# jyakaranda/A-LeGO-LOAM

Measured on AMD Instinct MI355X. Metric: scans/sec (16x1800 LiDAR) full IP->LO->LM loop, higher is better.
Workload: dtype f32/f64

## Files before the change

a-lego-loam_amd/csrc/kernels_lm.hip:

```cpp
#include <cstddef>
#include <cstring>

#include "../../include/alego_mi355x.h"
#include "dev_cost.h"
#include "nn_rules.h"
#include "remap_math.h"
#include "prof.h"
#include "kf_store.h"
#include "gmap.h"
#include "vgrid.h"
#include "vox_merge.h"

#define LM_BLOCK 256

DEV_INLINE double* ldp(const LmCtx& L, int slot) { return L.ld + (size_t)slot * LD_COUNT; }
DEV_INLINE int* lip(const LmCtx& L, int slot) { return L.li + (size_t)slot * LI_COUNT; }

DEV_INLINE void lm_map_update(const LmCtx& L, int slot, int* li, int merge) {
  const int nkf = li[LI_NKF];
  if (nkf == 0) return;
  int* rec = L.rec + (size_t)slot * L.K;
  const int cnt = li[LI_REC_CNT];
  bool changed = false;
  if (cnt < L.K) {
// ... 243 lines not shown
        int tot;
        const int e = noo + block_excl_scan<LT_T / 64>(oh ? 1 : 0, s_w, &tot);
        if (j < no) s_oop[j] = e;
        noo += tot;
      }
      if (tid == 0) s_oop[no] = noo;
      __syncthreads();
      vm_u64 kprev = c0 > 0 && c0 < c1 ? vkey_of(S[c0 - 1], inv) : 0;
      int hl = 0;
      for (int b0 = c0; b0 < c1; b0 += LT_B) {
        float4 p[LT_B + 1];
#pragma unroll
        for (int k = 0; k <= LT_B; ++k) p[k] = S[min(b0 + k, ns - 1)];
#pragma unroll
        for (int k = 0; k < LT_B; ++k) {
          const int i = b0 + k;
          if (i < c1) {
            const vm_u64 key = vkey_of(p[k], inv);
            if (i == 0 || kprev != key) {
              const int ol = vm_count_less(s_skey, no, key), ole = vm_count_le(s_skey, no, key);
              const int r = base + hl + s_oop[ol];
              ++hl;
              if (r < cap) {
                int nsr = 1;
                if (i + 1 < ns && vkey_of(p[k + 1], inv) == key) while (i + nsr < ns && vkey_of(S[i + nsr], inv) == key) ++nsr;
                out[r] = vm_centroid([&](int q) { return q == 0 ? p[k] : (q < nsr ? S[i + q] : O[s_idx[ol + q - nsr]]); }, 0, nsr + ole - ol);
              }
            }
            kprev = key;
          }
        }
      }
      for (int j = tid; j < no; j += LT_T) {
        if (s_osb[j] >= 0 && (j == 0 || s_skey[j - 1] != s_skey[j])) {
          const int r = s_base[s_osb[j] >> 16] + (s_osb[j] & 0xFFFF) + s_oop[j];
          if (r < cap) {
            int e = j + 1;
            while (e < no && s_skey[e] == s_skey[j]) ++e;
            out[r] = vm_centroid([&](int q) { return O[s_idx[q]]; }, j, e);
          }
        }
      }
      const int nvox = nsh + noo;
      if (tid == 0) { li[LI_NTOTAL] = n; li[LI_NTOTAL_DS] = min(nvox, cap); if (nvox > cap) li[LI_OVERFLOW] = 1; li[LI_TM_FAST] += 1; }
    } else {
      float4* t = L.cur_total + (size_t)slot * L.total_cap;
      for (int i = tid; i < ns; i += LT_T) t[i] = S[i];
      for (int i = tid; i < no; i += LT_T) t[ns + i] = O[i];
      if (tid == 0) { li[LI_NTOTAL] = n; li[LI_TM_LIST] += 1; }
      state = n > W.small_max ? 2 : 1;
    }
  }
  if (tid == 0) {
    if (state == 1) W.list_small[atomicAdd(&W.cnt[0], 1)] = slot - L.vox_slot0;
    else if (state == 2) W.list_big[atomicAdd(&W.cnt[1], 1)] = slot - L.vox_slot0;
    if (blockIdx.x == 0) { W.cnt_next[0] = 0; W.cnt_next[1] = 0; }
  }
}

DEV_INLINE int grid_cell(const GridGeom& g, float x, float y, float z, int* cx, int* cy, int* cz) {
  *cx = nn_lm_coord(x, g.inv) - g.ox; *cy = nn_lm_coord(y, g.inv) - g.oy; *cz = nn_lm_coord(z, g.inv) - g.oz;
  return nn_lm_index(*cx, *cy, *cz, g.gx, g.gy, g.gz);
}

__global__ void __launch_bounds__(LM_BLOCK) lm_grid_build(DevCtx d, LmCtx L) {
  const int slot = blockIdx.y + d.slot0, m = blockIdx.x;
  const int* li = lip(L, slot);
  if (!li[LI_REBUILD]) return;
  __shared__ GridGeom s_g;
  __shared__ int s[LM_BLOCK / 64];
  __shared__ int s_run;
  if (threadIdx.x == 0) {
    const unsigned* bb = d.opt_map_merge ? L.map_bbox + ((size_t)slot * 2 + m) * 8 : L.vox_bbox + ((size_t)(slot - L.vox_slot0) * 2 + m) * 8;
    GridGeom g;
    float mn[3], mx[3];
    vgr_box_load(bb, mn, mx);
    if (li[LI_KRAW_C + m] <= 0) { for (int a = 0; a < 3; ++a) { mn[a] = 0.f; mx[a] = 0.f; } }
    float cell = nn_lm_cell(d.P.knn_max_dist);
    int lo[3], hi[3];
    for (;;) {
      for (int a = 0; a < 3; ++a) { lo[a] = nn_lm_coord(mn[a], 1.0f / cell) - 1; hi[a] = nn_lm_coord(mx[a], 1.0f / cell) + 1; }
      const long long ex = (long long)hi[0] - lo[0] + 1, ey = (long long)hi[1] - lo[1] + 1, ez = (long long)hi[2] - lo[2] + 1;
      if (ex <= L.gcap && ey <= L.gcap && ez <= L.gcap && ex * ey * ez <= (long long)L.gcap) { g.gx = (int)ex; g.gy = (int)ey; g.gz = (int)ez; break; }
      cell *= 2.0f;
    }
    g.ox = lo[0]; g.oy = lo[1]; g.oz = lo[2]; g.inv = 1.0f / cell; g.ncell = g.gx * g.gy * g.gz;
    s_g = g;
    L.grid[(size_t)slot * 2 + m] = g;
    s_run = 0;
  }
  __syncthreads();
  const GridGeom g = s_g;
  const int ncell = g.ncell;
  int* cs = L.cell_start + ((size_t)slot * 2 + m) * (L.gcap + 1);
  int* cc = L.cell_cur + ((size_t)slot * 2 + m) * (L.gcap + 1);
  for (int c = threadIdx.x; c <= ncell; c += LM_BLOCK) cs[c] = 0;
  __threadfence_block();
  __syncthreads();
  const int n = li[LI_KDS_C + m];
  const float4* pts = (m == 0 ? L.map_corner_ds + (size_t)slot * L.map_cap_c : L.map_surf_ds + (size_t)slot * L.map_cap_s);
  float4* cp = L.cell_pts + ((size_t)slot * 2 + m) * L.map_cap_s;
  for (int i = threadIdx.x; i < n; i += LM_BLOCK) {
    const float4 p = pts[i];
    int cx, cy, cz;
    atomicAdd(&cs[grid_cell(g, p.x, p.y, p.z, &cx, &cy, &cz)], 1);
  }
  __threadfence_block();
  __syncthreads();
  for (int c0 = 0; c0 <= ncell; c0 += LM_BLOCK) {
    const int c = c0 + threadIdx.x;
    const int v = __hip_atomic_load(&cs[min(c, ncell)], __ATOMIC_RELAXED, __HIP_MEMORY_SCOPE_AGENT) * (c < ncell ? 1 : 0);
    int tot;
    const int ex = block_excl_scan<LM_BLOCK / 64>(v, s, &tot);
    const int run = s_run;
    if (c <= ncell) { const int e2 = run + ex; cs[c] = e2; cc[c] = e2; }
    __syncthreads();
    if (threadIdx.x == 0) s_run = run + tot;
  }
  __threadfence_block();
  __syncthreads();
  for (int i = threadIdx.x; i < n; i += LM_BLOCK) {
    const float4 p = pts[i];
    int cx, cy, cz;
    const int pos = atomicAdd(&cc[grid_cell(g, p.x, p.y, p.z, &cx, &cy, &cz)], 1);
    cp[pos] = make_float4(p.x, p.y, p.z, __int_as_float(i));
  }
}

DEV_INLINE void d_eig3(const double Ain[9], double lam[3], double vmax[3], double* lam_mid) {
  double A[9], V[9];
#pragma unroll
  for (int i = 0; i < 9; ++i) { A[i] = Ain[i]; V[i] = (i % 4 == 0) ? 1.0 : 0.0; }
  for (int sweep = 0; sweep < 60; ++sweep) {
    const double off = A[1] * A[1] + A[2] * A[2] + A[5] * A[5];
    if (off < 1e-300) break;
    if (off <= 1e-40 * (A[0] * A[0] + A[4] * A[4] + A[8] * A[8])) break;
#pragma unroll
    for (int p = 0; p < 2; ++p)
#pragma unroll
      for (int q = p + 1; q < 3; ++q) {
        const double apq = A[p * 3 + q];
        if (apq == 0.0) continue;
        const double theta = (A[q * 3 + q] - A[p * 3 + p]) / (2.0 * apq);
        const double t = (theta >= 0 ? 1.0 : -1.0) / (fabs(theta) + sqrt(theta * theta + 1.0));
        const double c = 1.0 / sqrt(t * t + 1.0), s = t * c;
#pragma unroll
        for (int k = 0; k < 3; ++k) { const double akp = A[k * 3 + p], akq = A[k * 3 + q]; A[k * 3 + p] = c * akp - s * akq; A[k * 3 + q] = s * akp + c * akq; }
#pragma unroll
        for (int k = 0; k < 3; ++k) { const double apk = A[p * 3 + k], aqk = A[q * 3 + k]; A[p * 3 + k] = c * apk - s * aqk; A[q * 3 + k] = s * apk + c * aqk; }
#pragma unroll
        for (int k = 0; k < 3; ++k) { const double vkp = V[k * 3 + p], vkq = V[k * 3 + q]; V[k * 3 + p] = c * vkp - s * vkq; V[k * 3 + q] = s * vkp + c * vkq; }
      }
  }
  const double dd[3] = {A[0], A[4], A[8]};
  int imax = 0, imin = 0;
  if (dd[1] > dd[imax]) imax = 1;
  if (dd[2] > dd[imax]) imax = 2;
  if (dd[1] < dd[imin]) imin = 1;
  if (dd[2] < dd[imin]) imin = 2;
  int imid = 3 - imax - imin;
  if (imax == imin) { imax = 2; imin = 0; imid = 1; }
  lam[0] = dd[imin]; lam[1] = dd[imid]; lam[2] = dd[imax];
  *lam_mid = dd[imid];
  vmax[0] = V[0 * 3 + imax]; vmax[1] = V[1 * 3 + imax]; vmax[2] = V[2 * 3 + imax];
}

DEV_INLINE void d_colpiv_qr53(double A[3][5], const double b[5], double x[3]) {
  const double eps = 2.220446049250313e-16, tiny = 2.2250738585072014e-308;
  double nu[3], nd[3], hc[3], c[5];
  int perm[3] = {0, 1, 2};
  double maxn = 0;
#pragma unroll
  for (int k = 0; k < 3; ++k) {
    double s2 = 0;
#pragma unroll
    for (int i = 0; i < 5; ++i) s2 += A[k][i] * A[k][i];
    nd[k] = nu[k] = sqrt(s2);
    if (nu[k] > maxn) maxn = nu[k];
  }
  const double threshold_helper = (maxn * eps) * (maxn * eps) / 5.0;
  const double downdate_threshold = 1.4901161193847656e-08;
  int nonzero = 3;
#pragma unroll
  for (int k = 0; k < 3; ++k) {
    int big = k;
    double nbig = nu[k];
#pragma unroll
    for (int j = k + 1; j < 3; ++j) if (nu[j] > nbig) { big = j; nbig = nu[j]; }
    if (nonzero == 3 && nbig * nbig < threshold_helper * (double)(5 - k)) nonzero = k;
#pragma unroll
    for (int j = k + 1; j < 3; ++j)
      if (big == j) {
#pragma unroll
        for (int i = 0; i < 5; ++i) { const double t = A[k][i]; A[k][i] = A[j][i]; A[j][i] = t; }
        { const double t = nu[k]; nu[k] = nu[j]; nu[j] = t; }
        { const double t = nd[k]; nd[k] = nd[j]; nd[j] = t; }
        { const int t = perm[k]; perm[k] = perm[j]; perm[j] = t; }
      }
    double tail2 = 0;
#pragma unroll
    for (int i = k + 1; i < 5; ++i) tail2 += A[k][i] * A[k][i];
    const double c0 = A[k][k];
    double beta, tau;
    if (tail2 <= tiny) {
      tau = 0; beta = c0;
#pragma unroll
      for (int i = k + 1; i < 5; ++i) A[k][i] = 0;
    } else {
      beta = sqrt(c0 * c0 + tail2);
      if (c0 >= 0) beta = -beta;
#pragma unroll
      for (int i = k + 1; i < 5; ++i) A[k][i] = A[k][i] / (c0 - beta);
      tau = (beta - c0) / beta;
    }
    hc[k] = tau;
    A[k][k] = beta;
    if (tau != 0) {
#pragma unroll
      for (int j = k + 1; j < 3; ++j) {
        double t = 0;
#pragma unroll
        for (int i = k + 1; i < 5; ++i) t += A[k][i] * A[j][i];
        t += A[j][k];
        A[j][k] -= tau * t;
#pragma unroll
        for (int i = k + 1; i < 5; ++i) A[j][i] -= tau * A[k][i] * t;
      }
    }
#pragma unroll
    for (int j = k + 1; j < 3; ++j) {
      if (nu[j] != 0) {
        double t = fabs(A[j][k]) / nu[j];
        t = (1.0 + t) * (1.0 - t);
        t = t < 0 ? 0 : t;
        const double q = nu[j] / nd[j];
        const double t2 = t * (q * q);
        if (t2 <= downdate_threshold) {
          double s2 = 0;
#pragma unroll
          for (int i = k + 1; i < 5; ++i) s2 += A[j][i] * A[j][i];
          nd[j] = nu[j] = sqrt(s2);
        } else nu[j] *= sqrt(t);
      }
    }
  }
#pragma unroll
  for (int i = 0; i < 5; ++i) c[i] = b[i];
#pragma unroll
  for (int k = 0; k < 3; ++k) {
    const double tau = hc[k];
    if (k < nonzero && tau != 0) {
      double t = 0;
#pragma unroll
      for (int i = k + 1; i < 5; ++i) t += A[k][i] * c[i];
      t += c[k];
      c[k] -= tau * t;
#pragma unroll
      for (int i = k + 1; i < 5; ++i) c[i] -= tau * A[k][i] * t;
    }
  }
#pragma unroll
  for (int k = 2; k >= 0; --k) {
    if (k < nonzero) {
      double sum = c[k];
#pragma unroll
      for (int j = k + 1; j < 3; ++j) if (j < nonzero) sum -= A[j][k] * c[j];
      c[k] = sum / A[k][k];
    } else c[k] = 0.0;
  }
#pragma unroll
  for (int o = 0; o < 3; ++o) {
    double v = 0.0;
#pragma unroll
    for (int i = 0; i < 3; ++i) if (perm[i] == o) v = c[i];
    x[o] = v;
  }
}

#ifndef LM_KNN_LANES
#define LM_KNN_LANES 4
#endif

DEV_INLINE void lm_shard_slice(const LmCtx& L, int nqc, int nqs, int kind, int* qlo, int* qhi) {
  int lo = 0, hi = nqc + nqs;
  if (L.shard_world > 1) {
    const long long T = nqc + nqs;
    lo = (int)(T * L.shard_rank / L.shard_world); hi = (int)(T * (L.shard_rank + 1) / L.shard_world);
  }
  if (kind == 0) { *qlo = min(lo, nqc); *qhi = min(hi, nqc); } else { *qlo = max(lo - nqc, 0); *qhi = max(hi - nqc, 0); }
}

DEV_INLINE bool lm_reg_block(const DevCtx& d, int GX, int* slot, int* kind, int* bx) {
  const int per = 2 * GX, b = blockIdx.x, oct = b / (8 * per), r = b - oct * 8 * per;
  const int s = oct * 8 + (r & 7), w = r >> 3;
  *slot = s + d.slot0; *kind = w / GX; *bx = w - (w / GX) * GX;
  return s < d.n_launch;
}
static inline int lm_reg_grid(const DevCtx& d, int GX) { return ((d.n_launch + 7) / 8) * 8 * 2 * GX; }

#define LM_ASSOC_GX 64
#ifndef LM_KNN_PK
#define LM_KNN_PK 1
#endif
__global__ void __launch_bounds__(128) lm_knn(DevCtx d, LmCtx L) {
  int slot, kind, bx;
  if (!lm_reg_block(d, LM_ASSOC_GX, &slot, &kind, &bx)) return;
  const int gx = LM_ASSOC_GX;
  const int* li = lip(L, slot);
  if (!li[LI_RUN]) return;
  const alego_params& P = d.P;
  if (lm_reg_skipped(li, P)) return;
  const int nq = kind == 0 ? li[LI_NCUR_C] : li[LI_NTOTAL_DS];
  int qlo, qhi;
  lm_shard_slice(L, li[LI_NCUR_C], li[LI_NTOTAL_DS], kind, &qlo, &qhi);
  const float4* qp = kind == 0 ? L.cur_corner_ds + (size_t)slot * L.kf_cap_c : L.cur_total_ds + (size_t)slot * L.total_cap;
  const int nmap = li[LI_KDS_C + kind];
  const GridGeom g = L.grid[(size_t)slot * 2 + kind];
  const int* cs = L.cell_start + ((size_t)slot * 2 + kind) * (L.gcap + 1);
  const float4* cp = L.cell_pts + ((size_t)slot * 2 + kind) * L.map_cap_s;
  const double* ld = ldp(L, slot);
  const DQuat qm = ldq(ld + LD_Q_M2L);
  constexpr int QPB = 128 / LM_KNN_LANES;
  const int sub = threadIdx.x & (LM_KNN_LANES - 1);
  const uint32_t limbits = nn_lm_limit_bits(P.knn_max_dist);
  const int nq_round = (nq + QPB - 1) / QPB * QPB;
  for (int qq = bx * QPB + threadIdx.x / LM_KNN_LANES; qq < nq_round; qq += gx * QPB) {
  const int q = min(qq, nq - 1);
  const float4 pin = qp[q];
  const double vin[3] = {pin.x, pin.y, pin.z};
  double r[3];
  dq_rotate(qm, vin, r);
  const float sx = (float)(r[0] + ld[LD_T_M2L + 0]), sy = (float)(r[1] + ld[LD_T_M2L + 1]), sz = (float)(r[2] + ld[LD_T_M2L + 2]);
  typedef nn_key_t u64k;
  const u64k KNONE = NN_NONE;
  u64k k0 = KNONE, k1 = KNONE, k2 = KNONE, k3 = KNONE, k4 = KNONE, kmax = KNONE;
  if (nmap >= 5 && q >= qlo && q < qhi) {
    int cx, cy, cz;
    grid_cell(g, sx, sy, sz, &cx, &cy, &cz);
    int rs[9], re[9];
#pragma unroll
    for (int r = 0; r < 9; ++r) {
      const int z = cz + r / 3 - 1, y = cy + r % 3 - 1;
      const int x0 = max(cx - 1, 0), x1 = min(cx + 1, g.gx - 1);
      const bool in = z >= 0 && z < g.gz && y >= 0 && y < g.gy && x0 <= x1;
      const int c0 = x0 + g.gx * (y + g.gy * z), c1 = x1 + g.gx * (y + g.gy * z);
      const int a0 = cs[in ? c0 : 0], a1 = cs[in ? c1 + 1 : 0];
      rs[r] = in ? a0 : 0;
      re[r] = in ? a1 : 0;
    }
    const nn_v2f sxy = {sx, sy};
    auto consider = [&](const float4& a) {
#if LM_KNN_PK
      const float dist = nn_d2_pk(sxy, sz, nn_v2f{a.x, a.y}, a.z);
#else
      const float dist = nn_d2(sx, sy, sz, a.x, a.y, a.z);
#endif
      const u64k key = nn_key(dist, (uint32_t)__float_as_int(a.w));
      if (key < kmax && nn_lm_within(dist, limbits)) {
        const bool e0 = k0 == kmax, e1 = !e0 && k1 == kmax, e2 = !e0 && !e1 && k2 == kmax, e3 = !e0 && !e1 && !e2 && k3 == kmax, e4 = !e0 && !e1 && !e2 && !e3;
        k0 = e0 ? key : k0; k1 = e1 ? key : k1; k2 = e2 ? key : k2; k3 = e3 ? key : k3; k4 = e4 ? key : k4;
        const u64k m01 = k0 > k1 ? k0 : k1, m23 = k2 > k3 ? k2 : k3, m03 = m01 > m23 ? m01 : m23;
        kmax = m03 > k4 ? m03 : k4;
      }
    };
    float4 first[9];
#pragma unroll
    for (int r = 0; r < 9; ++r) first[r] = cp[rs[r] + sub < re[r] ? rs[r] + sub : 0];
#ifndef LM_KNN_ORDER
#define LM_KNN_ORDER 1
#endif
    constexpr int ord[9] = {4, 1, 3, 5, 7, 0, 2, 6, 8};
#pragma unroll
    for (int k = 0; k < 9; ++k) { const int r = LM_KNN_ORDER ? ord[k] : k; if (rs[r] + sub < re[r]) consider(first[r]); }
#pragma unroll
    for (int k = 0; k < 9; ++k) {
      const int r = LM_KNN_ORDER ? ord[k] : k;
      for (int t = rs[r] + sub + LM_KNN_LANES; t < re[r]; t += 2 * LM_KNN_LANES) {
        const int t1 = t + LM_KNN_LANES;
        const float4 a0 = cp[t], a1 = cp[t1 < re[r] ? t1 : t];
        consider(a0);
        if (t1 < re[r]) consider(a1);
      }
    }
  }
  float bd[5];
  int bi[5];
  {
#pragma unroll
    for (int k = 0; k < 5; ++k) {
      const u64k m01 = k0 < k1 ? k0 : k1, m23 = k2 < k3 ? k2 : k3, m03 = m01 < m23 ? m01 : m23, mine = m03 < k4 ? m03 : k4;
      const u64k m = group_min_u64<LM_KNN_LANES>(mine);
      bd[k] = nn_key_d2(m); bi[k] = nn_key_index(m);
      if (mine == m && m != KNONE) {
        k0 = k0 == m ? KNONE : k0; k1 = k1 == m ? KNONE : k1; k2 = k2 == m ? KNONE : k2; k3 = k3 == m ? KNONE : k3; k4 = k4 == m ? KNONE : k4;
      }
    }
  }
  if (sub == 0 && qq < nq) {
    int* kn = lm_knn_of(L, slot, kind, q);
    const bool ok = nn_lm_row_ok(bi[4], bd[4], P.knn_max_dist) && q >= qlo && q < qhi;
#pragma unroll
    for (int k = 0; k < 5; ++k) kn[k] = ok ? bi[k] : -1;
  }
  }
}

#define LM_FIT_GX 20
__global__ void __launch_bounds__(128) lm_fit(DevCtx d, LmCtx L) {
  int slot, kind, bx;
  if (!lm_reg_block(d, LM_FIT_GX, &slot, &kind, &bx)) return;
  const int gx = LM_FIT_GX;
  const int* li = lip(L, slot);
  if (!li[LI_RUN]) return;
  const alego_params& P = d.P;
  if (lm_reg_skipped(li, P)) return;
  const int nq = kind == 0 ? li[LI_NCUR_C] : li[LI_NTOTAL_DS];
  const float4* mp = kind == 0 ? L.map_corner_ds + (size_t)slot * L.map_cap_c : L.map_surf_ds + (size_t)slot * L.map_cap_s;
  for (int q = bx * 128 + threadIdx.x; q < nq; q += gx * 128) {
  const int* kn = lm_knn_of(L, slot, kind, q);
  double* blk = lm_blocks_of(L, slot) + lm_row_of(kind, q, L.kf_cap_c) * LMB_W;
  int bi[5];
#pragma unroll
  for (int k = 0; k < 5; ++k) bi[k] = kn[k];
  lmb_put_none(blk);
  do {
    if (bi[0] < 0) break;
  if (kind == 0) {
    double near[5][3], center[3] = {0, 0, 0};
#pragma unroll
    for (int j = 0; j < 5; ++j) {
      const float4 m = mp[bi[j]];
      near[j][0] = m.x; near[j][1] = m.y; near[j][2] = m.z;
#pragma unroll
      for (int a = 0; a < 3; ++a) center[a] = center[a] + near[j][a];
    }
#pragma unroll
    for (int a = 0; a < 3; ++a) center[a] = center[a] / 5.0;
    double cov[9] = {0, 0, 0, 0, 0, 0, 0, 0, 0};
#pragma unroll
    for (int j = 0; j < 5; ++j) {
      const double zm[3] = {near[j][0] - center[0], near[j][1] - center[1], near[j][2] - center[2]};
#pragma unroll
      for (int a = 0; a < 3; ++a)
#pragma unroll
        for (int b = 0; b < 3; ++b) cov[a * 3 + b] = cov[a * 3 + b] + zm[a] * zm[b];
    }
    double lam[3], v[3], lmid;
    d_eig3(cov, lam, v, &lmid);
    if (lam[2] > P.line_ratio * lam[1]) {
      double pa[3], pb[3];
#pragma unroll
      for (int a = 0; a < 3; ++a) { pa[a] = P.line_half_len * v[a] + center[a]; pb[a] = -P.line_half_len * v[a] + center[a]; }
      lmb_put_edge(blk, pa, pb);
    }
  } else {
    double A[3][5], b[5], nrm[3];
    float mx[5], my[5], mz[5];
#pragma unroll
    for (int j = 0; j < 5; ++j) {
      const float4 m = mp[bi[j]];
      mx[j] = m.x; my[j] = m.y; mz[j] = m.z;
      A[0][j] = m.x; A[1][j] = m.y; A[2][j] = m.z; b[j] = -1.0;
    }
    d_colpiv_qr53(A, b, nrm);
    const double nn = sqrt(nrm[0] * nrm[0] + nrm[1] * nrm[1] + nrm[2] * nrm[2]);
    const double dd = 1 / nn;
#pragma unroll
    for (int a = 0; a < 3; ++a) nrm[a] /= nn;
    bool ok = true;
#pragma unroll
    for (int j = 0; j < 5; ++j)
      if (fabs(nrm[0] * mx[j] + nrm[1] * my[j] + nrm[2] * mz[j] + dd) > P.plane_tol) ok = false;
    if (ok) lmb_put_plane(blk, nrm, dd);
  }
  } while (false);
  }
}

#ifndef LM_SOLVE_T
#define LM_SOLVE_T 256
#endif
#define LM_SOLVE_RED_BYTES ((size_t)28 * (LM_SOLVE_T / 8) * sizeof(double))
#define LM_SOLVE_DYN_BYTES ((size_t)158 * 1024)
#define LM_SOLVE_ROW_BYTES_DEFAULT ((size_t)96 * 1024)
template <int T>
DEV_INLINE void lm_pack_rows(const LmCtx& L, int slot, int nqc, int nqs, unsigned char* row_lds, size_t row_budget, int (*s_cnt)[T / 64], LmRows& W) {
  const int tid = threadIdx.x, lane = tid & 63, wave = tid >> 6;
  const double* blocks = lm_blocks_of(L, slot);
  const float4* qc = L.cur_corner_ds + (size_t)slot * L.kf_cap_c;
  const float4* qs = L.cur_total_ds + (size_t)slot * L.total_cap;
  const int n_all = nqc + nqs, per = (n_all + T - 1) / T;
  const int lo = min(tid * per, n_all), hi = min(lo + per, n_all);
  auto block_of = [&](int i) { return blocks + lm_row_of_query(i, nqc, L.kf_cap_c) * LMB_W; };
  constexpr int U = 4;
  int cc = 0, cs = 0;
  for (int i0 = lo; i0 < hi; i0 += U) {
    double ty[U];
#pragma unroll
    for (int u = 0; u < U; ++u) ty[u] = block_of(min(i0 + u, n_all - 1))[LMB_TYPE];
#pragma unroll
    for (int u = 0; u < U; ++u) if (i0 + u < hi && ty[u] != 0.0) { if (i0 + u < nqc) ++cc; else ++cs; }
  }
  const int ic = wave_incl_scan(cc), is = wave_incl_scan(cs);
  if (lane == 63) { s_cnt[0][wave] = ic; s_cnt[1][wave] = is; }
  __syncthreads();
  int epos = ic - cc, ppos = is - cs, Rc = 0, Rs = 0;
#pragma unroll
  for (int w = 0; w < T / 64; ++w) { const int a = s_cnt[0][w], b = s_cnt[1][w]; if (w < wave) { epos += a; ppos += b; } Rc += a; Rs += b; }
  W = lml_make(Rc, Rs, row_lds, row_budget, lm_crows_of(L, slot));
  for (int i0 = lo; i0 < hi; i0 += U) {
    LmBlock B[U];
    float4 pt[U];
#pragma unroll
    for (int u = 0; u < U; ++u) {
      const int i = min(i0 + u, n_all - 1);
      B[u] = lmb_load(block_of(i));
      pt[u] = i < nqc ? qc[i] : qs[i - nqc];
    }
#pragma unroll
    for (int u = 0; u < U; ++u) {
      const int i = i0 + u;
      if (i < hi && lmb_type(B[u]) != 0.0) {
        const bool is_c = i < nqc;
        const int r = is_c ? epos++ : ppos++;
        if (is_c && r < W.Ce) lml_put_edge(W, r, B[u], pt[u]);
        else if (!is_c && r < W.Cp) lml_put_plane(W, r, B[u], pt[u]);
        else lms_put(W.crows + (is_c ? lms_edge_at(r) : lms_plane_at(Rc, r)) * LMS_W, B[u], pt[u]);
      }
    }
  }
  __threadfence_block();
  __syncthreads();
}

template <int T, bool FULL = true>
DEV_INLINE void lm_eval_rows(const LmRows& W, const PoseTerms& Tm, double huber, double acc[28]) {
  const double c3[3] = {0, 0, 0};
  for (int i = threadIdx.x; i < W.Rc; i += T) {
    LmEdge e;
    if (i < W.Ce) e = lml_edge(W, i); else e = lms_edge(W.crows + lms_edge_at(i) * LMS_W);
    if constexpr (FULL) {
      double res, J[6];
      eval_block(BLK_EDGE, e.p, e.a, e.b, c3, 0.0, Tm, &res, J);
      accumulate_block(res, J, huber, acc);
    } else accumulate_cost(eval_block_residual<BLK_EDGE>(e.p, e.a, e.b, c3, 0.0, Tm), huber, acc[27]);
  }
  for (int j = threadIdx.x; j < W.Rs; j += T) {
    LmPlane p;
    if (j < W.Cp) p = lml_plane(W, j); else p = lms_plane(W.crows + lms_plane_at(W.Rc, j) * LMS_W);
    if constexpr (FULL) {
      double res, J[6];
      eval_block(BLK_PLANE, p.p, p.n, c3, c3, p.d, Tm, &res, J);
      accumulate_block(res, J, huber, acc);
    } else accumulate_cost(eval_block_residual<BLK_PLANE>(p.p, p.n, c3, c3, p.d, Tm), huber, acc[27]);
  }
}

struct ShflHip { DEV_INLINE double operator()(double v, int src) const { return __shfl(v, src); } };
struct ShflDirect {
  DEV_INLINE double operator()(double v, int src) const {
    const long long b = __double_as_longlong(v);
    const int lo = __builtin_amdgcn_ds_bpermute(src << 2, (int)(unsigned)(unsigned long long)b), hi = __builtin_amdgcn_ds_bpermute(src << 2, (int)(unsigned)((unsigned long long)b >> 32));
    return __longlong_as_double((long long)(((unsigned long long)(unsigned)hi << 32) | (unsigned)lo));
  }
};
template <class Shfl>
DEV_INLINE double rc_eigen_lanes(double A, int i, int j, double lam[6], const Shfl& shfl) {
  double V = i == j ? 1.0 : 0.0;
  for (int sweep = 0; sweep < RC_SWEEPS_MAX; ++sweep) {
    double off = 0.0, dg = 0.0;
#pragma unroll
    for (int a = 0; a < 6; ++a)
#pragma unroll
      for (int b = a + 1; b < 6; ++b) { const double x = shfl(A, a * 6 + b); off += x * x; }
#pragma unroll
    for (int a = 0; a < 6; ++a) { const double x = shfl(A, a * 7); dg += x * x; }
    if (!(off > RC_OFF_REL * dg)) break;
#pragma unroll
    for (int pp = 0; pp < 5; ++pp)
#pragma unroll
      for (int q = pp + 1; q < 6; ++q) {
        const double apq = shfl(A, pp * 6 + q);
        if (apq == 0.0) continue;
        double c, s;
        rc_rot_cs(shfl(A, pp * 7), shfl(A, q * 7), apq, &c, &s);
        { const double xp = shfl(A, i * 6 + pp), xq = shfl(A, i * 6 + q); A = rc_rot_col(j, pp, q, c, s, xp, xq, A); }
        { const double xp = shfl(A, pp * 6 + j), xq = shfl(A, q * 6 + j); A = rc_rot_row(i, pp, q, c, s, xp, xq, A); }
        { const double xp = shfl(V, i * 6 + pp), xq = shfl(V, i * 6 + q); V = rc_rot_col(j, pp, q, c, s, xp, xq, V); }
      }
  }
  double dd[6];
  int rk[6], src = 0;
#pragma unroll
  for (int k = 0; k < 6; ++k) dd[k] = shfl(A, k * 7);
#pragma unroll
  for (int k = 0; k < 6; ++k) { rk[k] = rc_rank(dd, k); if (rk[k] == j) src = k; }
#pragma unroll
  for (int r = 0; r < 6; ++r) {
    double v = 0.0;
#pragma unroll
    for (int k = 0; k < 6; ++k) v = rk[k] == r ? dd[k] : v;
    lam[r] = v;
  }
  return shfl(V, i * 6 + src);
}

template <class Shfl>
DEV_INLINE int rc_front_lanes(const double* s_out , const double* t6, const double* p, int n_edge, int n_plane, double* s_N , int lane, int i, int j,
                              const Shfl& shfl, double* info, double* vs, double lam[6], double vi[6], double vj[6]) {
  if (n_edge + n_plane <= 6) return 0;
  if (fabs(t6[3]) < RC_COS_PITCH_MIN) return -3;
  {
    double N[36];
    rc_minv_t(t6, N);
    double v = 0.0;
#pragma unroll
    for (int k = 0; k < 36; ++k) v = lane == k ? N[k] : v;
    if (lane < 36) s_N[lane] = v;
    __threadfence_block();
  }
  __builtin_amdgcn_sched_barrier(0);
  *info = rc_info_entry(s_out, s_N, i < j ? i : j, i < j ? j : i);
  const bool bad = !rc_finite(*info) || (lane < 28 && !rc_finite(s_out[lane])) || (lane < 6 && !rc_finite(p[lane]));
  if (__any(bad)) return -2;
  __builtin_amdgcn_sched_barrier(0);
  *vs = rc_eigen_lanes(*info, i, j, lam, shfl);
  __builtin_amdgcn_sched_barrier(0);
#pragma unroll
  for (int k = 0; k < 6; ++k) { vi[k] = shfl(*vs, i * 6 + k); vj[k] = shfl(*vs, j * 6 + k); }
  return 1;
}
template <class Header> DEV_INLINE void rec_store_empty(double* dv, int count, const double* head, int keep, int lane, Header&& header) {
  for (int k = lane; k < count; k += 64) dv[k] = k < keep ? head[k] : 0.0;
  if (lane == 0) header();
}

struct RmLds {
  double P[36], N[36], M[36];
  double eig_min;
  alego_remap* rec;
  int on, first, n_edge, n_plane, frame;
};
static_assert(offsetof(alego_remap, start) == 16 && sizeof(alego_remap) == 16 + 84 * sizeof(double), "rm_empty hands rec_store_empty the record's doubles from `start`");
template <bool REMAP> DEV_INLINE RmLds* rm_lds() {
  if constexpr (REMAP) { __shared__ RmLds R; return &R; }
  else return nullptr;
}
DEV_INLINE void rm_header(alego_remap* rec, int status, int n_held, int frame) { rec->status = status; rec->n_held = n_held; rec->frame = frame; rec->pad = 0; }
DEV_INLINE void rm_empty(alego_remap* rec, int status, int frame, const double* x0, int lane) { rec_store_empty(rec->start, 84, x0, 6, lane, [&] { rm_header(rec, status, 0, frame); }); }
DEV_INLINE void rm_tail(const double* s_out , const double* s_trig , RmLds& R, const double* x0, int n_edge, int n_plane, int frame, double eig_min, alego_remap* rec) {
  int lane = threadIdx.x;
  asm volatile("" : "+v"(lane));
  const int l = lane < 36 ? lane : 35, i = l / 6, j = l - 6 * i;
  const double t6[6] = {s_trig[7], s_trig[6], s_trig[9], s_trig[8], s_trig[11], s_trig[10]};
  if (lane == 0) { R.on = 0; R.first = 0; }
  double info, vs, lam[6], vi[6], vj[6], col[6];
  const ShflDirect shfl;
  const int st = rc_front_lanes(s_out, t6, x0, n_edge, n_plane, R.N, lane, i, j, shfl, &info, &vs, lam, vi, vj);
  if (st != 1) { rm_empty(rec, st, frame, x0, lane); return; }
  __builtin_amdgcn_sched_barrier(0);
  {
    double M[36];
    rc_m_t(t6, M);
    double v = 0.0;
#pragma unroll
    for (int k = 0; k < 36; ++k) v = lane == k ? M[k] : v;
    if (lane < 36) R.M[lane] = v;
    __threadfence_block();
  }
  __builtin_amdgcn_sched_barrier(0);
  const double pt = rm_pt_entry(vi, vj, lam, eig_min);
#pragma unroll
  for (int a = 0; a < 6; ++a) {
    double row[6];
#pragma unroll
    for (int b = 0; b < 6; ++b) row[b] = shfl(pt, a * 6 + b);
    col[a] = rm_ptm_entry(row, R.M, j);
    __builtin_amdgcn_sched_barrier(0);
  }
  int held = 0;
  double lam_j = 0.0;
  bool bad = false;
#pragma unroll
  for (int k = 0; k < 6; ++k) { bad = bad || !rc_finite(lam[k]); held += rm_kept(lam[k], eig_min) ? 0 : 1; lam_j = j == k ? lam[k] : lam_j; }
  const double pe = rm_p_entry(R.N, i, col);
  const double P = held == 0 ? (i == j ? 1.0 : 0.0) : (held == 6 ? 0.0 : pe);
// ... 410 lines not shown
```

Before: 498,500.

## Buffer kNN candidates in per-lane LDS queue and drain in batches

Reworks the LM kNN inner loop so candidate keys are no longer inserted into the register top-5 on every point. Each lane writes its key unconditionally to an LDS queue and advances a counter only for valid in-range hits. The queue is drained into the top-5 when any lane in the wave nears capacity, with a bulk fill when the set is empty. The aim is to remove the divergent branchy insert from the hot loop, at the cost of 8 KB of LDS per workgroup, extra LDS traffic, and wave-wide drains that may reduce occupancy.

```diff
diff --git a/a-lego-loam_amd/csrc/kernels_lm.hip b/a-lego-loam_amd/csrc/kernels_lm.hip
--- a/a-lego-loam_amd/csrc/kernels_lm.hip
+++ b/a-lego-loam_amd/csrc/kernels_lm.hip
@@ -569,7 +569,17 @@
 #ifndef LM_KNN_PK
 #define LM_KNN_PK 1
 #endif
+#ifndef LM_KNN_QUEUE
+#define LM_KNN_QUEUE 1
+#endif
+#ifndef LM_KNN_QCAP
+#define LM_KNN_QCAP 8
+#endif
+static_assert(LM_KNN_QCAP >= 8 && LM_KNN_QCAP <= 16, "LM_KNN_QCAP: 8 .. 16 entries per lane (1 KB of LDS per entry and workgroup)");
 __global__ void __launch_bounds__(128) lm_knn(DevCtx d, LmCtx L) {
+#if LM_KNN_QUEUE
+  __shared__ nn_key_t lm_knn_q[LM_KNN_QCAP][128];
+#endif
   int slot, kind, bx;
   if (!lm_reg_block(d, LM_ASSOC_GX, &slot, &kind, &bx)) return;
   const int gx = LM_ASSOC_GX;
@@ -616,19 +626,54 @@
       re[r] = in ? a1 : 0;
     }
     const nn_v2f sxy = {sx, sy};
-    auto consider = [&](const float4& a) {
-#if LM_KNN_PK
+    auto replace_max = [&](const u64k key) {
+      const bool e0 = k0 == kmax, e1 = !e0 && k1 == kmax, e2 = !e0 && !e1 && k2 == kmax, e3 = !e0 && !e1 && !e2 && k3 == kmax, e4 = !e0 && !e1 && !e2 && !e3;
+      k0 = e0 ? key : k0; k1 = e1 ? key : k1; k2 = e2 ? key : k2; k3 = e3 ? key : k3; k4 = e4 ? key : k4;
+      const u64k m01 = k0 > k1 ? k0 : k1, m23 = k2 > k3 ? k2 : k3, m03 = m01 > m23 ? m01 : m23;
+      kmax = m03 > k4 ? m03 : k4;
+    };
+#if LM_KNN_QUEUE
+    int qn = 0;
+    auto drain = [&]() {
+      int i = 0;
+      if (k0 == KNONE) {
+        const u64k v0 = lm_knn_q[0][threadIdx.x], v1 = lm_knn_q[1][threadIdx.x], v2 = lm_knn_q[2][threadIdx.x], v3 = lm_knn_q[3][threadIdx.x], v4 = lm_knn_q[4][threadIdx.x];
+        k0 = qn > 0 ? v0 : KNONE; k1 = qn > 1 ? v1 : KNONE; k2 = qn > 2 ? v2 : KNONE; k3 = qn > 3 ? v3 : KNONE; k4 = qn > 4 ? v4 : KNONE;
+        const u64k m01 = k0 > k1 ? k0 : k1, m23 = k2 > k3 ? k2 : k3, m03 = m01 > m23 ? m01 : m23;
+        kmax = m03 > k4 ? m03 : k4;
+        i = 5;
+      }
+      for (; i < qn; ++i) {
+        const u64k key = lm_knn_q[i][threadIdx.x];
+        if (key < kmax) replace_max(key);
+      }
+      qn = 0;
+    };
+    auto room = [&](const int n) { if (__builtin_amdgcn_ballot_w64(qn > LM_KNN_QCAP - n) != 0) drain(); };
+#endif
+    auto consider = [&](const float4& a, const bool valid) {
+#if LM_KNN_QUEUE
+#else
+      if (!valid) return;
+#endif
+#if LM_KNN_QUEUE
+      float az = a.z;
+      asm volatile("" : "+v"(az));
+      const float dist0 = nn_d2_pk(sxy, sz, nn_v2f{a.x, a.y}, az);
+      float dist = dist0;
+      asm volatile("" : "+v"(dist));
+#elif LM_KNN_PK
       const float dist = nn_d2_pk(sxy, sz, nn_v2f{a.x, a.y}, a.z);
 #else
       const float dist = nn_d2(sx, sy, sz, a.x, a.y, a.z);
 #endif
       const u64k key = nn_key(dist, (uint32_t)__float_as_int(a.w));
-      if (key < kmax && nn_lm_within(dist, limbits)) {
-        const bool e0 = k0 == kmax, e1 = !e0 && k1 == kmax, e2 = !e0 && !e1 && k2 == kmax, e3 = !e0 && !e1 && !e2 && k3 == kmax, e4 = !e0 && !e1 && !e2 && !e3;
-        k0 = e0 ? key : k0; k1 = e1 ? key : k1; k2 = e2 ? key : k2; k3 = e3 ? key : k3; k4 = e4 ? key : k4;
-        const u64k m01 = k0 > k1 ? k0 : k1, m23 = k2 > k3 ? k2 : k3, m03 = m01 > m23 ? m01 : m23;
-        kmax = m03 > k4 ? m03 : k4;
-      }
+#if LM_KNN_QUEUE
+      lm_knn_q[qn][threadIdx.x] = key;
+      qn += valid && nn_lm_within(dist, limbits) ? 1 : 0;
+#else
+      if (key < kmax && nn_lm_within(dist, limbits)) replace_max(key);
+#endif
     };
     float4 first[9];
 #pragma unroll
@@ -638,17 +683,29 @@
 #endif
     constexpr int ord[9] = {4, 1, 3, 5, 7, 0, 2, 6, 8};
 #pragma unroll
-    for (int k = 0; k < 9; ++k) { const int r = LM_KNN_ORDER ? ord[k] : k; if (rs[r] + sub < re[r]) consider(first[r]); }
+    for (int k = 0; k < 9; ++k) {
+      const int r = LM_KNN_ORDER ? ord[k] : k;
+#if LM_KNN_QUEUE
+      if (k >= LM_KNN_QCAP) room(1);
+#endif
+      consider(first[r], rs[r] + sub < re[r]);
+    }
 #pragma unroll
     for (int k = 0; k < 9; ++k) {
       const int r = LM_KNN_ORDER ? ord[k] : k;
       for (int t = rs[r] + sub + LM_KNN_LANES; t < re[r]; t += 2 * LM_KNN_LANES) {
         const int t1 = t + LM_KNN_LANES;
         const float4 a0 = cp[t], a1 = cp[t1 < re[r] ? t1 : t];
-        consider(a0);
-        if (t1 < re[r]) consider(a1);
-      }
-    }
+#if LM_KNN_QUEUE
+        room(2);
+#endif
+        consider(a0, true);
+        consider(a1, t1 < re[r]);
+      }
+    }
+#if LM_KNN_QUEUE
+    drain();
+#endif
   }
   float bd[5];
   int bi[5];
```

Result: no change. 503,300, median of 6 (+1.0%).
